# MartinPippel/DAmar

Measured on AMD Instinct MI355X. Metric: aligned base-pairs/sec (daligner block-vs-block), higher is better.
Workload: dtype int32

## Files before the change

damar_amd/csrc/kernels/seed_merge.hip:

```cpp
#include "dev_common.h"
#include "kernels.h"

SEED_PRIO_VAR(g_merge_prio, 0)
SEED_PRIO_SETTER(damar_merge_set_prio, g_merge_prio)


__device__ __forceinline__ u32 count_below(const u32 *__restrict__ bpos, u32 jb, u32 ib, u32 bound)
{ u32 a = jb, b = ib;
  while (a < b)
    { u32 m = (a + b) >> 1;
      if (bpos[m] < bound) a = m + 1; else b = m;
    }
  return a - jb;
}


#ifndef MT_PER
#define MT_PER  4
#endif
#define MT_A    (MT_PER * 256)
#define MT_BCAP (3 * MT_A)
#define MT_HITS 4
#define MT_NBK  2048

// ... 1172 lines not shown
              }
        }
      else
        {
#pragma unroll
          for (int y = 0; y < q; y++)
            prev = (d[y] == d[q]) ? c[y] : prev;
        }
      add[q] = min(c[q] - prev, kmer);
    }
  if (UNS && top > SCREEN_PANEL)
    return true;
  bool ok = false;
#pragma unroll
  for (int x = 0; x < N; x++)
    { int sum = 0;
#pragma unroll
      for (int y = 0; y < N; y++)
        sum += ((u32) (d[y] - d[x]) <= 1u) ? add[y] : 0;
      ok |= (x < n) && (sum >= hitmin);
    }
  return ok;
}

template <bool UNS>
__global__ __launch_bounds__(256)
void pair_work_mark(const u64 *__restrict__ keys, const u32 *__restrict__ vals, u64 nhits, int ppos, int dbits, int abits,
                    int minhit, int nshift, const u64 *__restrict__ send, int binshift, int kmer, int hitmin,
                    u32 b_lo, u32 b_hi, u64 *__restrict__ bits, u32 *__restrict__ tcount)
{ SEED_PRIO(g_merge_prio);
  __shared__ u64 sk[DAMAR_SCAN_TILE + PW_HALO + 1];
  __shared__ u64 bb[(PH_ROUNDS + 1) * 4];
  __shared__ u16 hl[DAMAR_SCAN_TILE];
  __shared__ u16 cl[DAMAR_SCAN_TILE];
  __shared__ u32 kb[DAMAR_SCAN_TILE / 32];
  __shared__ u32 bl[DAMAR_SCAN_TILE / PW_SMALL];
  __shared__ u32 nh, nlo, nhi, nb;
  const int  pshift = ppos + dbits;
  const u64  pmask = (1ull << ppos) - 1;
  const int  nthr = nshift < 0 ? 0 : 1 << nshift;
  const int  l = lane_id(), w = threadIdx.x >> 6;
  const u64  base = (u64) blockIdx.x * DAMAR_SCAN_TILE;
  {
    constexpr int NLD = (DAMAR_SCAN_TILE + PW_HALO + 1 + 255) / 256;
    u64 v[NLD];
#pragma unroll
    for (int q = 0; q < NLD; q++)
      { u64 i = base + (u64) q * 256u + threadIdx.x;
        i = i > 0 ? i - 1 : 0;
        v[q] = keys[i < nhits ? i : nhits - 1];
      }
#pragma unroll
    for (int q = 0; q < NLD; q++)
      { const u32 j = (u32) q * 256u + threadIdx.x;
        if (j < DAMAR_SCAN_TILE + PW_HALO + 1)
          sk[j] = v[q];
      }
  }
  if (threadIdx.x < DAMAR_SCAN_TILE / 32)
    kb[threadIdx.x] = 0;
  if (threadIdx.x == 0)
    nh = nlo = nhi = nb = 0;
  u64 e0 = ~0ull, e1 = ~0ull;
  for (int t = 0; t < nthr; t++)
    { const u64 e = send[t];
      if (e > base)
        { e0 = e;
          if (t + 1 < nthr)
            e1 = send[t + 1];
          break;
        }
    }
  __syncthreads();

  u64 mk[PH_ROUNDS];
  u32 tot = 0;
#pragma unroll
  for (int r = 0; r <= PH_ROUNDS; r++)
    { const u32 off = (u32) r * 256u + threadIdx.x;
      const u64 i = base + off;
      bool st = true, f = false;
      if (i < nhits && off < DAMAR_SCAN_TILE + PW_HALO)
        { const u64 pr = sk[off + 1] >> pshift;
          const u64 ip = i + (u64) (minhit - 1);
          st = (i == 0) || (sk[off] >> pshift) != pr;
          if (r < PH_ROUNDS && st && ip < nhits)
            { const u64 kp = (minhit - 1 <= PW_HALO) ? sk[off + (u32) minhit] : keys[ip];
              if ((kp >> pshift) == pr)
                { f = true;
                  if (i < e0)
                    { if (i + (u64) minhit >= e0) f = false; }
                  else if (i < e1)
                    { if (i + (u64) minhit >= e1) f = false; }
                  else
                    for (int t = 0; t < nthr; t++)
                      { u64 e = send[t];
                        if (i < e)
                          { if (i + (u64) minhit >= e) f = false;
                            break;
                          }
                      }
                }
            }
        }
      const u64 ms = __ballot(st);
      if (l == 0)
        bb[r * 4 + w] = ms;
      if (r < PH_ROUNDS)
        { mk[r] = __ballot(f);
          tot += (u32) __popcll(mk[r]);
        }
    }
  if (tot != 0)
    { u32 at = 0;
      if (l == 0)
        at = atomicAdd(&nh, tot);
      at = (u32) __shfl((int) at, 0);
#pragma unroll
      for (int r = 0; r < PH_ROUNDS; r++)
        { if ((mk[r] >> l) & 1)
            hl[at + (u32) __popcll(mk[r] & lanes_below(l))] = (u16) ((u32) r * 256u + threadIdx.x);
          at += (u32) __popcll(mk[r]);
        }
    }
  __syncthreads();

  const u32 nheads = nh;
  for (u32 h0 = 0; h0 < nheads; h0 += 256)
    { const u32 h = h0 + threadIdx.x;
      u32 off = 0;
      int n = 0, kind = 0;
      if (h < nheads)
        { off = hl[h];
          const u32 rb = (u32) ((sk[off + 1] >> pshift) >> abits);
          if (rb >= b_lo && rb < b_hi)
            { const u32 p = off + 1;
              u64 ws = bb[p >> 6] >> (p & 63);
              if (p & 63)
                ws |= bb[(p >> 6) + 1] << (64 - (p & 63));
              n = ws ? __ffsll((long long) ws) : 65;
              if (n > SCREEN_MAX || minhit > SCREEN_MAX ||
                  (!UNS && (int) ((sk[off + (u32) n] >> dbits) & pmask) > SCREEN_PANEL))
                atomicOr(&kb[off >> 5], 1u << (off & 31));
              else if (n > PW_SMALL)
                bl[atomicAdd(&nb, 1u)] = off | ((u32) n << 16);
              else
                kind = n > PW_SHORT ? 2 : 1;
            }
        }
      const u64 m1 = __ballot(kind == 1), m2 = __ballot(kind == 2);
      u32 a1 = 0, a2 = 0;
      if (l == 0)
        { if (m1) a1 = atomicAdd(&nlo, (u32) __popcll(m1));
          if (m2) a2 = atomicAdd(&nhi, (u32) __popcll(m2));
        }
      a1 = (u32) __shfl((int) a1, 0);
      a2 = (u32) __shfl((int) a2, 0);
      if (kind == 1)
        cl[a1 + (u32) __popcll(m1 & lanes_below(l))] = (u16) (off | ((u32) n << 12));
      else if (kind == 2)
        cl[DAMAR_SCAN_TILE - 1 - (a2 + (u32) __popcll(m2 & lanes_below(l)))] = (u16) (off | ((u32) n << 12));
    }
  __syncthreads();

  const u32 n_lo = nlo, n_hi = nhi;
  const u32 lo_rounds = (n_lo + 255u) & ~255u;
  for (u32 h0 = 0; h0 < lo_rounds + n_hi; h0 += 256)
    { const u32 h = h0 + threadIdx.x;
      const bool act = h0 < lo_rounds ? h < n_lo : h - lo_rounds < n_hi;
      const u32 e = act ? (u32) cl[h0 < lo_rounds ? h : DAMAR_SCAN_TILE - 1 - (h - lo_rounds)] : 0u;
      const u32 off = e & 0xfffu;
      const int n = act ? (int) (e >> 12) : 0;
      bool keep = false;
      if (dbits == 0)
        { const u64 i = base + off;
          int dlast = 0x7fffffff;
          for (int x = 0; x < n && !keep; x++)
            { const int dx = (int) vals[i + (u64) x] >> binshift;
              if (dx == dlast)
                continue;
              dlast = dx;
              int s0 = 0, s1 = 0, p0 = 0, p1 = 0;
              for (int y = 0; y < n; y++)
                { const int dy = (int) vals[i + (u64) y] >> binshift;
                  const int ap = (int) ((sk[off + 1 + (u32) y] >> dbits) & pmask);
                  if (dy == dx)
                    { s0 += (ap - p0 >= kmer) ? kmer : ap - p0;  p0 = ap; }
                  else if (dy == dx + 1)
                    { s1 += (ap - p1 >= kmer) ? kmer : ap - p1;  p1 = ap; }
                }
              keep = s0 + s1 >= hitmin;
            }
        }
      else if (__ballot(n > 0) != 0)
        { if      (__ballot(n > 7) != 0) keep = pw_screen_small<8, UNS>(sk + off + 1, n, pmask, dbits, binshift, kmer, hitmin);
          else if (__ballot(n > 6) != 0) keep = pw_screen_small<7, UNS>(sk + off + 1, n, pmask, dbits, binshift, kmer, hitmin);
          else if (__ballot(n > 5) != 0) keep = pw_screen_small<6, UNS>(sk + off + 1, n, pmask, dbits, binshift, kmer, hitmin);
          else if (__ballot(n > 4) != 0) keep = pw_screen_small<5, UNS>(sk + off + 1, n, pmask, dbits, binshift, kmer, hitmin);
          else if (__ballot(n > 3) != 0) keep = pw_screen_small<4, UNS>(sk + off + 1, n, pmask, dbits, binshift, kmer, hitmin);
          else                           keep = pw_screen_small<3, UNS>(sk + off + 1, n, pmask, dbits, binshift, kmer, hitmin);
        }
      if (keep)
        atomicOr(&kb[off >> 5], 1u << (off & 31));
    }
  const u32 nbig = nb;
  for (u32 q = threadIdx.x >> 6; q < nbig; q += 4)
    { const u32 off = bl[q] & 0xffffu;
      const int n = (int) (bl[q] >> 16);
      const u64 i = base + off;
      const int xl = l < n ? l : n - 1;
      const int dx = seed_diag(sk[off + 1 + (u32) xl], vals, i + (u64) xl, pmask, dbits) >> binshift;
      if (UNS)
        {
          const int apx = (int) ((sk[off + 1 + (u32) xl] >> dbits) & pmask);
          int prev = 0, top = 0;
          for (int y = 0; y < n; y++)
            { const u64 ky = sk[off + 1 + (u32) y];
              const int dy = seed_diag(ky, vals, i + (u64) y, pmask, dbits) >> binshift;
              const int ap = (int) ((ky >> dbits) & pmask);
              const bool before = ap < apx || (ap == apx && y < xl);
              prev = (dy == dx && before && ap > prev) ? ap : prev;
              top = ap > top ? ap : top;
            }
          const int addx = (l < n) ? min(apx - prev, kmer) : 0;
          int sum = 0;
          for (int y = 0; y < n; y++)
            { const int ay = __shfl(addx, y), dy = __shfl(dx, y);
              sum += ((u32) (dy - dx) <= 1u) ? ay : 0;
            }
          if ((top > SCREEN_PANEL || __ballot(l < n && sum >= hitmin) != 0) && l == 0)
            atomicOr(&kb[off >> 5], 1u << (off & 31));
          continue;
        }
      int s0 = 0, s1 = 0, p0 = 0, p1 = 0;
#pragma unroll 4
      for (int y = 0; y < n; y++)
        { const u64 ky = sk[off + 1 + (u32) y];
          const int dy = seed_diag(ky, vals, i + (u64) y, pmask, dbits) >> binshift;
          const int ap = (int) ((ky >> dbits) & pmask);
          if (dy == dx)
            { s0 += (ap - p0 >= kmer) ? kmer : ap - p0;  p0 = ap; }
          else if (dy == dx + 1)
            { s1 += (ap - p1 >= kmer) ? kmer : ap - p1;  p1 = ap; }
        }
      if (__ballot(s0 + s1 >= hitmin) != 0 && l == 0)
        atomicOr(&kb[off >> 5], 1u << (off & 31));
    }
  __syncthreads();
  if (threadIdx.x < 64)
    { const u64 m = (u64) kb[2 * threadIdx.x] | ((u64) kb[2 * threadIdx.x + 1] << 32);
      bits[(base >> 6) + threadIdx.x] = m;
      const int c = wave_incl_scan_i(__popcll(m));
      if (threadIdx.x == 63)
        tcount[blockIdx.x] = (u32) c;
    }
}

#define OR_MAX   2048
#define OR_WAVE  512
#define OR_SLICE 32
__device__ __forceinline__ u32 run_length(const u64 *keys, u64 nhits, u64 i, int pshift, u32 maxrun, int l, u64 pr)
{ u32 n = 0;
  for (;;)
    { const u64 x = i + (u64) n + (u64) l;
      const u64 same = __ballot(x < nhits && (keys[x] >> pshift) == pr);
      if (same != ~0ull)
        return n + (u32) __ffsll((long long) ~same) - 1u;
      n += 64;
      if (n > maxrun)
        return n;
    }
}

__global__ __launch_bounds__(256)
void order_probe(const u64 *__restrict__ keys, u64 nhits, int ppos, int dbits, const u64 *__restrict__ bits, u64 *__restrict__ flag,
                 u32 maxrun)
{ SEED_PRIO(g_merge_prio);
  __shared__ u16 hl[DAMAR_SCAN_TILE];
  __shared__ u32 nh;
  const int  l = lane_id();
  const u64  base = (u64) blockIdx.x * DAMAR_SCAN_TILE;
  if (threadIdx.x == 0)
    nh = 0;
  __syncthreads();
  if (threadIdx.x < DAMAR_SCAN_TILE / 64)
    { u64 w = bits[(base >> 6) + threadIdx.x];
      while (w)
        { const int b = __ffsll((long long) w) - 1;
          w &= w - 1;
          hl[atomicAdd(&nh, 1u)] = (u16) (threadIdx.x * 64u + (u32) b);
        }
    }
  __syncthreads();
  const u32 n_h = nh;
  bool over = false;
  for (u32 h = threadIdx.x >> 6; h < n_h; h += 4)
    { const u64 i = base + hl[h];
      over |= run_length(keys, nhits, i, ppos + dbits, maxrun, l, keys[i] >> (ppos + dbits)) > maxrun;
    }
  if (over && l == 0)
    atomicOr((unsigned long long *) flag, 1ull);
}

template <u32 J>
__device__ __forceinline__ u32 lane_xor(u32 v)
{ if constexpr (J == 1)
    return (u32) __builtin_amdgcn_update_dpp(0, (int) v, 0xB1, 0xf, 0xf, true);
  else if constexpr (J == 2)
    return (u32) __builtin_amdgcn_update_dpp(0, (int) v, 0x4E, 0xf, 0xf, true);
  else if constexpr (J == 8)
    return (u32) __builtin_amdgcn_update_dpp(0, (int) v, 0x128, 0xf, 0xf, true);
  else if constexpr (J == 4 || J == 16)
    return (u32) __builtin_amdgcn_ds_swizzle((int) v, (int) (0x1f | (J << 10)));
  else
    return (u32) __shfl_xor((int) v, (int) J);
}

template <int K, u32 K2, u32 JJ>
__device__ __forceinline__ void or_step(u32 (&c)[K], int l)
{ if constexpr (JJ >= 64)
    {
#pragma unroll
      for (int q = 0; q < K; q++)
        if ((q & (int) (JJ >> 6)) == 0)
          { const int  p  = q | (int) (JJ >> 6);
            const bool up = (((u32) q << 6) & K2) == 0;
            const u32  lo = min(c[q], c[p]), hi = max(c[q], c[p]);
            c[q] = up ? lo : hi;
            c[p] = up ? hi : lo;
          }
    }
  else
    {
#pragma unroll
      for (int q = 0; q < K; q++)
        { const u32  o  = lane_xor<JJ>(c[q]);
          const bool up = (((u32) q * 64u + (u32) l) & K2) == 0;
          c[q] = (up == (((u32) l & JJ) == 0)) ? min(c[q], o) : max(c[q], o);
        }
    }
}

template <int K, u32 K2, u32 JJ>
__device__ __forceinline__ void or_merge(u32 (&c)[K], int l)
{ or_step<K, K2, JJ>(c, l);
  if constexpr (JJ > 1)
    or_merge<K, K2, JJ / 2>(c, l);
}

template <int K, u32 K2>
__device__ __forceinline__ void or_network(u32 (&c)[K], int l)
{ if constexpr (K2 > 2)
    or_network<K, K2 / 2>(c, l);
  or_merge<K, K2, K2 / 2>(c, l);
}

template <int K>
__device__ __forceinline__ void or_sort_regs(u64 *keys, u64 i, u32 n, int dbits, u64 pmask, int l)
{ u32 c[K];
#pragma unroll
  for (int q = 0; q < K; q++)
    { const u32 j = (u32) q * 64u + (u32) l;
      c[q] = (j < n) ? (((u32) ((keys[i + j] >> dbits) & pmask) << 11) | j) : 0xffffffffu;
    }
  or_network<K, 64u * K>(c, l);
  u64 v[K];
#pragma unroll
  for (int q = 0; q < K; q++)
    { const u32 j = (u32) q * 64u + (u32) l;
      v[q] = keys[i + ((j < n) ? (c[q] & 2047u) : 0u)];
    }
  asm volatile("s_waitcnt vmcnt(0)" ::: "memory");
#pragma unroll
  for (int q = 0; q < K; q++)
    { const u32 j = (u32) q * 64u + (u32) l;
      if (j < n)
        keys[i + j] = v[q];
    }
}

#ifdef OR_STATS
static __device__ unsigned long long g_or_hist[16];
#endif

__global__ __launch_bounds__(256)
void order_waves(u64 *keys, u64 nhits, int ppos, int dbits, const u32 *__restrict__ work, u32 nwork, u32 slice,
                 u32 *__restrict__ lcount, u32 *__restrict__ llist)
{ SEED_PRIO(g_merge_prio);
  const int  l = lane_id(), pshift = ppos + dbits;
  const u64  pmask = (1ull << ppos) - 1;
  const u32  first = blockIdx.x * slice;
  const u32  end = min(first + slice, nwork);
  for (u32 t = first + (threadIdx.x >> 6); t < end; t += 4)
    { const u64 i = work[t];
      const u64 x = i + (u64) l;
      const u64 k0 = keys[x < nhits ? x : nhits - 1];
      const u64 pr = (u64) __shfl((long long) (k0 >> pshift), 0);
      const u64 same = __ballot(x < nhits && (k0 >> pshift) == pr);
      u32 n;
      if (same != ~0ull)
        n = (u32) __ffsll((long long) ~same) - 1u;
      else
        n = 64u + run_length(keys, nhits, i + 64u, pshift, OR_MAX - 64u, l, pr);
#ifdef OR_STATS
      if (l == 0)
        { int b = 0;
          while (b < 12 && (2u << b) < n) b += 1;
          atomicAdd(&g_or_hist[n > OR_MAX ? 12 : b], 1ull);
          atomicAdd(&g_or_hist[13], (unsigned long long) n);
        }
#endif
      if (n < 2)
        continue;
      if (n <= 64)
        { u32 c[1] = { (u32) l < n ? (((u32) ((k0 >> dbits) & pmask) << 11) | (u32) l) : 0xffffffffu };
          or_network<1, 64u>(c, l);
          const int src = (int) (c[0] & 63u);
          const u32 lo = (u32) __shfl((int) (u32) k0, src), hi = (u32) __shfl((int) (u32) (k0 >> 32), src);
          if ((u32) l < n)
            keys[x] = ((u64) hi << 32) | lo;
        }
      else if (n <= 128)
        or_sort_regs<2>(keys, i, n, dbits, pmask, l);
      else if (n <= 256)
        or_sort_regs<4>(keys, i, n, dbits, pmask, l);
      else if (n <= OR_WAVE)
        or_sort_regs<8>(keys, i, n, dbits, pmask, l);
      else if (n <= OR_MAX && l == 0)
        { const u32 at = atomicAdd(lcount, 1u);
          llist[2 * at] = (u32) i;
          llist[2 * at + 1] = n;
        }
    }
}

__global__ __launch_bounds__(256)
void order_long(u64 *keys, int ppos, int dbits, const u32 *__restrict__ lcount, const u32 *__restrict__ llist)
{ SEED_PRIO(g_merge_prio);
  __shared__ u64 rk[OR_MAX];
  __shared__ u32 ck[OR_MAX];
  const u64  pmask = (1ull << ppos) - 1;
  const u32  nl = *lcount;
  for (u32 b = blockIdx.x; b < nl; b += gridDim.x)
    { const u64 i = llist[2 * b];
      const u32 n = llist[2 * b + 1];
      u32 P = 2;
      while (P < n)
        P <<= 1;
      for (u32 j = threadIdx.x; j < P; j += 256)
        { if (j < n)
            { const u64 k = keys[i + j];
              rk[j] = k;
              ck[j] = ((u32) ((k >> dbits) & pmask) << 11) | j;
            }
          else
            ck[j] = 0xffffffffu;
        }
      __syncthreads();
      for (u32 k2 = 2; k2 <= P; k2 <<= 1)
        for (u32 jj = k2 >> 1; jj > 0; jj >>= 1)
          { for (u32 t = threadIdx.x; t < (P >> 1); t += 256)
              { const u32 ix = ((t & ~(jj - 1)) << 1) | (t & (jj - 1)), px = ix | jj;
                const bool up = (ix & k2) == 0;
                const u32 a = ck[ix], c = ck[px];
                if ((a > c) == up)
                  { ck[ix] = c;  ck[px] = a; }
              }
            __syncthreads();
          }
      for (u32 j = threadIdx.x; j < n; j += 256)
        keys[i + j] = rk[ck[j] & 2047u];
      __syncthreads();
    }
}

size_t damar_order_runs_scratch_bytes(u64 nhits)
{ return sizeof(u32) * (size_t) (2 * (nhits / (OR_WAVE + 1)) + 2); }

#ifdef OR_STATS
static void or_stats_print(void)
{ unsigned long long h[16];
  if (hipMemcpyFromSymbol(h, HIP_SYMBOL(g_or_hist), sizeof(h)) != hipSuccess)
    return;
  unsigned long long runs = 0;
  for (int b = 0; b <= 12; b++)
    runs += h[b];
  fprintf(stderr, "order_runs: %llu kept runs, %llu seeds in them\n", runs, h[13]);
  for (int b = 0; b <= 12; b++)
    if (h[b])
      fprintf(stderr, "  runs of %5d..%-5d %9llu  (%.3f %%)\n", b == 0 ? 1 : (1 << b) + 1, b == 12 ? 1 << 30 : 2 << b, h[b], 100. * h[b] / runs);
}
#endif

void damar_launch_order_runs(u64 *keys, u64 nhits, int ppos, int dbits, const u32 *work, u32 nwork, void *scratch, hipStream_t st)
{ if (nwork == 0)
    return;
#ifdef OR_STATS
  static int reg = 0;
  if (!reg)
    { reg = 1;  atexit(or_stats_print); }
#endif
  u32 *lcount = (u32 *) scratch;
  HIP_CHECK(hipMemsetAsync(lcount, 0, sizeof(u32), st));
  const u32 slice = std::min<u32>(OR_SLICE, 4u * std::max<u32>(1u, nwork / 2048u));
  hipLaunchKernelGGL(order_waves, dim3((nwork + slice - 1) / slice), dim3(256), 0, st, keys, nhits, ppos, dbits, work, nwork, slice,
                     lcount, lcount + 2);
  if (nhits > OR_WAVE)
    { const u64 most = nhits / (OR_WAVE + 1);
      hipLaunchKernelGGL(order_long, dim3((u32) std::min<u64>(std::min<u64>(nwork, most), 1024)), dim3(256), 0, st, keys, ppos, dbits,
                         (const u32 *) lcount, (const u32 *) (lcount + 2));
    }
}

void damar_launch_pair_work(u64 *keys, const u32 *vals, u64 nhits, u64 off, u64 gtotal, int ppos, int dbits, int abits, int minhit, int nshift,
                            u64 *send, u64 *bits, void *scan_work, u64 *total_dev, int binshift, int kmer, int hitmin,
                            u32 b_lo, u32 b_hi, int unsorted, hipStream_t st)
{ HIP_CHECK(hipMemsetAsync(total_dev, 0, 2 * sizeof(u64), st));
  if (nhits == 0)
    return;
  if (nshift > 6)
    nshift = 6;
  const u32 ntiles = (u32) ((nhits + DAMAR_SCAN_TILE - 1) / DAMAR_SCAN_TILE);
  u32 *tcount = (u32 *) scan_work;
  if (nshift >= 0)
    hipLaunchKernelGGL(slice_ends<u64>, dim3(1), dim3(64), 0, st, keys, nhits, off, gtotal, abits + ppos + dbits, nshift, send);
  if (!unsorted)
    hipLaunchKernelGGL(pair_work_mark<false>, dim3(ntiles), dim3(256), 0, st, (const u64 *) keys, vals, nhits, ppos, dbits, abits, minhit,
                       nshift, (const u64 *) send, binshift, kmer, hitmin, b_lo, b_hi, bits, tcount);
  else
    { hipLaunchKernelGGL(pair_work_mark<true>, dim3(ntiles), dim3(256), 0, st, (const u64 *) keys, vals, nhits, ppos, dbits, abits, minhit,
                         nshift, (const u64 *) send, binshift, kmer, hitmin, b_lo, b_hi, bits, tcount);
      static int maxrun = -1;
      if (maxrun < 0)
        { const char *e = getenv("DAMAR_TEST_RUN_MAX");
          maxrun = (e && atoi(e) >= 2 && atoi(e) <= OR_MAX) ? atoi(e) : OR_MAX;
        }
      hipLaunchKernelGGL(order_probe, dim3(ntiles), dim3(256), 0, st, (const u64 *) keys, nhits, ppos, dbits, (const u64 *) bits, total_dev + 1,
                         (u32) maxrun);
    }
  damar_scan_tile_counts(tcount, ntiles, total_dev, st);
}

void damar_launch_pair_work_expand(const u64 *bits, const void *scan_work, u64 nhits, u32 *work, hipStream_t st)
{ if (nhits == 0)
    return;
  const u32 ntiles = (u32) ((nhits + DAMAR_SCAN_TILE - 1) / DAMAR_SCAN_TILE);
  hipLaunchKernelGGL(pair_heads_expand, dim3(ntiles), dim3(64), 0, st, bits, (const u32 *) scan_work, work);
}

__global__ __launch_bounds__(256)
void compact_u32(const u32 *__restrict__ src, const u32 *__restrict__ keep, const u32 *__restrict__ off, u32 n,
                 u32 *__restrict__ out)
{ u32 i = blockIdx.x * 256u + threadIdx.x;
  if (i < n && keep[i])
    out[off[i]] = src[i];
}

void damar_launch_compact_u32(const u32 *src, const u32 *keep, const u32 *off, u32 n, u32 *out, hipStream_t st)
{ if (n == 0)
    return;
  hipLaunchKernelGGL(compact_u32, dim3((n + 255) / 256), dim3(256), 0, st, src, keep, off, n, out);
}

__global__ __launch_bounds__(256)
void compact_index(const u32 *__restrict__ flags, const u32 *__restrict__ off, u64 n, u32 *__restrict__ out)
{ u64 i = (u64) blockIdx.x * 256u + threadIdx.x;
  if (i < n && flags[i])
    out[off[i]] = (u32) i;
}

void damar_launch_compact_index(const u32 *flags, const u32 *off, u64 n, u32 *out, hipStream_t st)
{ if (n == 0)
    return;
  hipLaunchKernelGGL(compact_index, dim3((u32) ((n + 255) / 256)), dim3(256), 0, st, flags, off, n, out);
}

__global__ __launch_bounds__(256)
void work_cost(const u64 *__restrict__ keys, const u32 *__restrict__ vals, u64 nhits, int pbits0, int abits, int dbits,
               const u32 *__restrict__ aboff, const u32 *__restrict__ bboff,
               const u32 *__restrict__ work, u32 nwork, u32 coarse, u32 *__restrict__ key, u32 *__restrict__ val)
{ u32 j = blockIdx.x * 256u + threadIdx.x;
  if (j >= nwork)
    return;
  const int pbits = pbits0 + dbits;
  const u64 i = work[j], pr = keys[i] >> pbits;
  u64 a = i + 1, b = (j + 1 < nwork) ? (u64) work[j + 1] : nhits;
  while (a < b)
    { u64 mid = (a + b) >> 1;
      if ((keys[mid] >> pbits) == pr) a = mid + 1; else b = mid;
    }
  u64 n = a - i;
  if (coarse >= 0xfffffffcu)
    { const u64 pm = (1ull << pbits0) - 1;
      const u64 ext = ((keys[a - 1] >> dbits) & pm) - ((keys[i] >> dbits) & pm);
      const u32 ra = (u32) (pr & ((1ull << abits) - 1)), rb = (u32) (pr >> abits);
      const int alen = (int) (aboff[ra + 1] - aboff[ra]) - 1, blen = (int) (bboff[rb + 1] - bboff[rb]) - 1;
      const int d = seed_diag(keys[i], vals, i, pm, dbits);
      const int geo = min(alen, blen + d) - max(0, d);
      u64 len = (coarse == 0xffffffffu) ? ext : (coarse == 0xfffffffeu ? (u64) max(geo, 0) : max(ext, (u64) max(geo, 0)));
      if (coarse == 0xfffffffcu)
        { const int xa0 = (int) ((keys[i] >> dbits) & pm), xb0 = xa0 - d;
          const int fw = min(alen - xa0, blen - xb0);
          len = (u64) max(fw, 0);
        }
      n = len >> (pbits0 > 16 ? pbits0 - 16 : 0);
      coarse = 0;
    }
  if (n > WORK_COST_MAX)
    n = WORK_COST_MAX;
  if (coarse == 1)
    key[j] = (u32) __clz((int) n) - (32 - WORK_COST_BITS);
  else
    key[j] = coarse ? (n >= coarse ? 0u : 1u) : (u32) (WORK_COST_MAX - n);
  val[j] = j;
}

void damar_launch_work_cost(const u64 *keys, const u32 *vals, u64 nhits, int pbits, int abits, int dbits, const u32 *aboff,
                            const u32 *bboff, const u32 *work, u32 nwork, u32 coarse, u32 *key, u32 *val, hipStream_t st)
{ if (nwork == 0)
    return;
  hipLaunchKernelGGL(work_cost, dim3((nwork + 255) / 256), dim3(256), 0, st, keys, vals, nhits, pbits, abits, dbits, aboff, bboff,
                     work, nwork, coarse, key, val);
}

void damar_preload_merge(void)
{ hipFuncAttributes fa;
  (void) hipFuncGetAttributes(&fa, (const void *) merge_emit);
}
```

Baseline: 53.83 billion.

## Fuse pair-work marking and run-length probe into one register-staged kernel

Adds a new kernel for the unsorted path that loads each wavefront's keys into registers and detects run boundaries with ballots. It stages the members of short runs into an LDS pool and screens them from there, and it folds the order/run-length overflow check that the separate order_probe kernel used to do into the same pass. This removes one kernel launch and a second sweep over keys and bits, and cuts repeated global reads during screening. The cost is heavy register and LDS use, with occupancy capped at six waves per EU, plus considerable new code that must match the old marking exactly. A fallback to the old two-kernel path remains when DAMAR_WORK_STAGED is set or dbits is zero.

```diff
diff --git a/damar_amd/csrc/kernels/seed_merge.hip b/damar_amd/csrc/kernels/seed_merge.hip
--- a/damar_amd/csrc/kernels/seed_merge.hip
+++ b/damar_amd/csrc/kernels/seed_merge.hip
@@ -1498,6 +1498,272 @@
     atomicOr((unsigned long long *) flag, 1ull);
 }
 
+#define PW_WSEEDS (DAMAR_SCAN_TILE / 4)
+#define PW_POOL   1792
+static_assert(PW_WSEEDS == PH_ROUNDS * 64 && PW_HALO == 64 && SCREEN_MAX < PW_HALO, "a wavefront's rounds and its halo round");
+
+__device__ __forceinline__ u64 lane_before(u64 v, u64 first)
+{ const u32 lo = (u32) __builtin_amdgcn_update_dpp((int) (u32) first, (int) (u32) v, 0x138, 0xf, 0xf, false);
+  const u32 hi = (u32) __builtin_amdgcn_update_dpp((int) (u32) (first >> 32), (int) (u32) (v >> 32), 0x138, 0xf, 0xf, false);
+  return ((u64) hi << 32) | lo;
+}
+
+__device__ __forceinline__ bool pw_screen_wave(const u64 *run, int n, int l, u64 pmask, int dbits, int binshift, int kmer, int hitmin)
+{ const u64 dmask = (1ull << dbits) - 1;
+  const int xl = l < n ? l : n - 1;
+  const u64 kx = run[xl];
+  const int apx = (int) ((kx >> dbits) & pmask);
+  const int dx = (apx - (int) (kx & dmask)) >> binshift;
+  int prev = 0, top = 0;
+  for (int y = 0; y < n; y++)
+    { const u64 ky = run[y];
+      const int ap = (int) ((ky >> dbits) & pmask);
+      const int dy = (ap - (int) (ky & dmask)) >> binshift;
+      const bool before = ap < apx || (ap == apx && y < xl);
+      prev = (dy == dx && before && ap > prev) ? ap : prev;
+      top = ap > top ? ap : top;
+    }
+  const int addx = (l < n) ? min(apx - prev, kmer) : 0;
+  int sum = 0;
+  for (int y = 0; y < n; y++)
+    { const int ay = __shfl(addx, y), dy = __shfl(dx, y);
+      sum += ((u32) (dy - dx) <= 1u) ? ay : 0;
+    }
+  return top > SCREEN_PANEL || __ballot(l < n && sum >= hitmin) != 0;
+}
+
+__device__ __forceinline__ bool pw_screen_lanes(const u64 *run, int n, u64 pmask, int dbits, int binshift, int kmer, int hitmin)
+{ if      (__ballot(n > 7) != 0) return pw_screen_small<8, true>(run, n, pmask, dbits, binshift, kmer, hitmin);
+  else if (__ballot(n > 6) != 0) return pw_screen_small<7, true>(run, n, pmask, dbits, binshift, kmer, hitmin);
+  else if (__ballot(n > 5) != 0) return pw_screen_small<6, true>(run, n, pmask, dbits, binshift, kmer, hitmin);
+  else if (__ballot(n > 4) != 0) return pw_screen_small<5, true>(run, n, pmask, dbits, binshift, kmer, hitmin);
+  else if (__ballot(n > 3) != 0) return pw_screen_small<4, true>(run, n, pmask, dbits, binshift, kmer, hitmin);
+  return pw_screen_small<3, true>(run, n, pmask, dbits, binshift, kmer, hitmin);
+}
+
+__global__ __launch_bounds__(256) __attribute__((amdgpu_waves_per_eu(6)))
+void pair_work_mark_regs(const u64 *__restrict__ keys, u64 nhits, int ppos, int dbits, int abits, int minhit, int nshift,
+                         const u64 *__restrict__ send, int binshift, int kmer, int hitmin, u32 b_lo, u32 b_hi,
+                         u64 *__restrict__ bits, u32 *__restrict__ tcount, u64 *__restrict__ flag, u32 maxrun)
+{ SEED_PRIO(g_merge_prio);
+  __shared__ u64 pool[PW_POOL];
+  __shared__ u64 mw[4][PH_ROUNDS + 1];
+  __shared__ u16 mp[4][PH_ROUNDS + 1];
+  __shared__ u16 cl[DAMAR_SCAN_TILE];
+  __shared__ u32 bl[DAMAR_SCAN_TILE / PW_SMALL];
+  __shared__ u32 kb[DAMAR_SCAN_TILE / 32];
+  __shared__ unsigned long long cnt;
+  __shared__ u32 inkeys[4];
+  const int  pshift = ppos + dbits;
+  const u64  pmask = (1ull << ppos) - 1;
+  const int  nthr = nshift < 0 ? 0 : 1 << nshift;
+  const int  l = lane_id(), w = threadIdx.x >> 6;
+  const u64  base = (u64) blockIdx.x * DAMAR_SCAN_TILE;
+  const u32  wb = (u32) w * PW_WSEEDS;
+  if (threadIdx.x == 0)
+    cnt = 0;
+  u64 e0 = ~0ull, e1 = ~0ull;
+  for (int t = 0; t < nthr; t++)
+    { const u64 e = send[t];
+      if (e > base)
+        { e0 = e;
+          if (t + 1 < nthr)
+            e1 = send[t + 1];
+          break;
+        }
+    }
+  __syncthreads();
+
+  u64 v[PH_ROUNDS + 1];
+#pragma unroll
+  for (int q = 0; q <= PH_ROUNDS; q++)
+    { const u64 i = base + wb + (u32) q * 64u + (u32) l;
+      v[q] = keys[i < nhits ? i : nhits - 1];
+    }
+  u64 ms[PH_ROUNDS + 1];
+  { const u64 ib = base + wb;
+    u64 last = keys[ib == 0 ? 0 : (ib - 1 < nhits ? ib - 1 : nhits - 1)];
+#pragma unroll
+    for (int q = 0; q <= PH_ROUNDS; q++)
+      { const u64 i = ib + (u32) q * 64u + (u32) l;
+        const u64 d = (v[q] ^ lane_before(v[q], last)) >> pshift;
+        ms[q] = __ballot(i >= nhits || i == 0 || d != 0);
+        last = bcast_u64(v[q], 63);
+      }
+  }
+
+  u32 code[(PH_ROUNDS + 1 + 3) / 4];
+  u32 n1 = 0, n2 = 0, n3 = 0, npool = 0;
+  u32 carry = 0;
+  bool over = false;
+#pragma unroll
+  for (int x = 0; x < (PH_ROUNDS + 1 + 3) / 4; x++)
+    code[x] = 0;
+#pragma unroll
+  for (int q = 0; q <= PH_ROUNDS; q++)
+    { u64 scr = 0;
+      u32 c = 0;
+      if (q < PH_ROUNDS)
+        { const u32 off = wb + (u32) q * 64u + (u32) l;
+          const u64 i = base + off;
+          u64 ws = ((ms[q] >> 1) >> l) | (ms[q + 1] << (63 - l));
+          const int n = ws ? __ffsll((long long) ws) : 65;
+          bool f = ((ms[q] >> l) & 1) && i < nhits && n >= (minhit - 1 > PW_HALO ? PW_HALO + 1 : minhit);
+          if (minhit - 1 > PW_HALO)
+            { const u64 ip = i + (u64) (minhit - 1);
+              f = f && ip < nhits;
+              if (f)
+                f = (keys[ip] >> pshift) == (v[q] >> pshift);
+            }
+          if (f)
+            { if (i < e0)
+                { if (i + (u64) minhit >= e0) f = false; }
+              else if (i < e1)
+                { if (i + (u64) minhit >= e1) f = false; }
+              else
+                for (int t = 0; t < nthr; t++)
+                  { u64 e = send[t];
+                    if (i < e)
+                      { if (i + (u64) minhit >= e) f = false;
+                        break;
+                      }
+                  }
+              const u32 rb = (u32) ((v[q] >> pshift) >> abits);
+              if (rb < b_lo || rb >= b_hi)
+                f = false;
+            }
+          const bool direct = f && (n > SCREEN_MAX || minhit > SCREEN_MAX);
+          const u64 kd = __ballot(direct);
+          if (l == 0)
+            { kb[(wb >> 5) + 2 * q] = (u32) kd;
+              kb[(wb >> 5) + 2 * q + 1] = (u32) (kd >> 32);
+            }
+          over |= direct && (u32) n > maxrun && (n <= 64 || maxrun < 64);
+          u64 lm = __ballot(direct && n > 64 && maxrun >= 64);
+          while (lm)
+            { const int b = __ffsll((long long) lm) - 1;
+              lm &= lm - 1;
+              const u64 ih = base + wb + (u32) q * 64u + (u32) b;
+              over |= run_length(keys, nhits, ih, pshift, maxrun, l, bcast_u64(v[q], b) >> pshift) > maxrun;
+            }
+          if (f && !direct)
+            c = (u32) n;
+          scr = __ballot(c != 0);
+          n1 += (u32) __popcll(__ballot(c != 0 && c <= PW_SHORT));
+          n2 += (u32) __popcll(__ballot(c > PW_SHORT && c <= PW_SMALL));
+          n3 += (u32) __popcll(__ballot(c > PW_SMALL));
+        }
+      const u64 a = ~(ms[q] & ~scr), s1 = a + scr, sum = s1 + carry;
+      const u32 cout = (s1 < a || sum < s1) ? 1u : 0u;
+      const u64 mem = ((sum ^ a ^ scr) >> 1) | ((u64) cout << 63);
+      carry = cout;
+      npool += (u32) __popcll(mem);
+      c |= (u32) ((mem >> l) & 1) << 7;
+      code[q >> 2] |= c << (8 * (q & 3));
+    }
+  if (__ballot(over) != 0 && l == 0)
+    atomicOr((unsigned long long *) flag, 1ull);
+
+  u32 a1, a2, a3, ap;
+  bool staged;
+  { unsigned long long at = 0;
+    if (l == 0)
+      at = atomicAdd(&cnt, (unsigned long long) n1 | ((unsigned long long) n2 << 16) | ((unsigned long long) n3 << 32) |
+                           ((unsigned long long) npool << 48));
+    at = bcast_u64(at, 0);
+    a1 = (u32) at & 0xffffu;  a2 = (u32) (at >> 16) & 0xffffu;  a3 = (u32) (at >> 32) & 0xffffu;  ap = (u32) (at >> 48);
+    staged = ap + npool <= PW_POOL;
+    if (l == 0)
+      inkeys[w] = staged ? 0u : 1u;
+  }
+  u64 my_mw = 0;
+  u32 my_mp = 0;
+#pragma unroll
+  for (int q = 0; q <= PH_ROUNDS; q++)
+    { const u32 c = (code[q >> 2] >> (8 * (q & 3))) & 0xffu;
+      const u32 n = c & 0x7fu, off = wb + (u32) q * 64u + (u32) l;
+      const u64 mem = __ballot((c & 0x80u) != 0);
+      if (l == q)
+        { my_mw = mem;  my_mp = ap; }
+      if (staged && (c & 0x80u))
+        pool[ap + (u32) __popcll(mem & lanes_below(l))] = v[q];
+      ap += (u32) __popcll(mem);
+      if (q < PH_ROUNDS)
+        { const u64 m1 = __ballot(n != 0 && n <= PW_SHORT), m2 = __ballot(n > PW_SHORT && n <= PW_SMALL), m3 = __ballot(n > PW_SMALL);
+          if (m1)
+            { if (n != 0 && n <= PW_SHORT)
+                cl[a1 + (u32) __popcll(m1 & lanes_below(l))] = (u16) (off | (n << 12));
+              a1 += (u32) __popcll(m1);
+            }
+          if (m2)
+            { if (n > PW_SHORT && n <= PW_SMALL)
+                cl[DAMAR_SCAN_TILE - 1 - (a2 + (u32) __popcll(m2 & lanes_below(l)))] = (u16) (off | (n << 12));
+              a2 += (u32) __popcll(m2);
+            }
+          if (m3)
+            { if (n > PW_SMALL)
+                bl[a3 + (u32) __popcll(m3 & lanes_below(l))] = off | (n << 16);
+              a3 += (u32) __popcll(m3);
+            }
+        }
+    }
+  if (l <= PH_ROUNDS)
+    { mw[w][l] = my_mw;
+      mp[w][l] = (u16) my_mp;
+    }
+  __syncthreads();
+
+  const unsigned long long tot = cnt;
+  const u32 n_lo = (u32) tot & 0xffffu, n_hi = (u32) (tot >> 16) & 0xffffu, nbig = (u32) (tot >> 32) & 0xffffu;
+  const u32 lo_rounds = (n_lo + 255u) & ~255u;
+  over = false;
+  for (u32 h0 = 0; h0 < lo_rounds + n_hi; h0 += 256)
+    { const u32 h = h0 + threadIdx.x;
+      const bool act = h0 < lo_rounds ? h < n_lo : h - lo_rounds < n_hi;
+      const u32 e = act ? (u32) cl[h0 < lo_rounds ? h : DAMAR_SCAN_TILE - 1 - (h - lo_rounds)] : 0u;
+      const u32 off = e & 0xfffu;
+      const int n = act ? (int) (e >> 12) : 0;
+      if (__ballot(n > 0) == 0)
+        continue;
+      const u32 hw = off >> 10, hq = (off >> 6) & (PH_ROUNDS - 1), hb = off & 63u;
+      bool keep;
+      if (__ballot(act && inkeys[hw] != 0) != 0)
+        keep = pw_screen_lanes(keys + base + off, n, pmask, dbits, binshift, kmer, hitmin);
+      else
+        keep = pw_screen_lanes(pool + (act ? (u32) mp[hw][hq] + (u32) __popcll(mw[hw][hq] & lanes_below((int) hb)) : 0u), n, pmask,
+                               dbits, binshift, kmer, hitmin);
+      if (keep)
+        { atomicOr(&kb[off >> 5], 1u << (off & 31));
+          over |= (u32) n > maxrun;
+        }
+    }
+  for (u32 q = threadIdx.x >> 6; q < nbig; q += 4)
+    { const u32 off = bl[q] & 0xffffu;
+      const int n = (int) (bl[q] >> 16);
+      const u32 hw = off >> 10, hq = (off >> 6) & (PH_ROUNDS - 1), hb = off & 63u;
+      bool keep;
+      if (inkeys[hw] != 0)
+        keep = pw_screen_wave(keys + base + off, n, l, pmask, dbits, binshift, kmer, hitmin);
+      else
+        keep = pw_screen_wave(pool + (u32) mp[hw][hq] + (u32) __popcll(mw[hw][hq] & lanes_below((int) hb)), n, l, pmask, dbits,
+                              binshift, kmer, hitmin);
+      if (keep && l == 0)
+        { atomicOr(&kb[off >> 5], 1u << (off & 31));
+          over |= (u32) n > maxrun;
+        }
+    }
+  if (__ballot(over) != 0 && l == 0)
+    atomicOr((unsigned long long *) flag, 1ull);
+  __syncthreads();
+  if (threadIdx.x < 64)
+    { const u64 m = (u64) kb[2 * threadIdx.x] | ((u64) kb[2 * threadIdx.x + 1] << 32);
+      bits[(base >> 6) + threadIdx.x] = m;
+      const int c = wave_incl_scan_i(__popcll(m));
+      if (threadIdx.x == 63)
+        tcount[blockIdx.x] = (u32) c;
+    }
+}
+
 template <u32 J>
 __device__ __forceinline__ u32 lane_xor(u32 v)
 { if constexpr (J == 1)
@@ -1724,15 +1990,22 @@
     hipLaunchKernelGGL(pair_work_mark<false>, dim3(ntiles), dim3(256), 0, st, (const u64 *) keys, vals, nhits, ppos, dbits, abits, minhit,
                        nshift, (const u64 *) send, binshift, kmer, hitmin, b_lo, b_hi, bits, tcount);
   else
-    { hipLaunchKernelGGL(pair_work_mark<true>, dim3(ntiles), dim3(256), 0, st, (const u64 *) keys, vals, nhits, ppos, dbits, abits, minhit,
-                         nshift, (const u64 *) send, binshift, kmer, hitmin, b_lo, b_hi, bits, tcount);
-      static int maxrun = -1;
+    { static int maxrun = -1;
+      static int staged = 0;
       if (maxrun < 0)
         { const char *e = getenv("DAMAR_TEST_RUN_MAX");
           maxrun = (e && atoi(e) >= 2 && atoi(e) <= OR_MAX) ? atoi(e) : OR_MAX;
-        }
-      hipLaunchKernelGGL(order_probe, dim3(ntiles), dim3(256), 0, st, (const u64 *) keys, nhits, ppos, dbits, (const u64 *) bits, total_dev + 1,
-                         (u32) maxrun);
+          staged = (e = getenv("DAMAR_WORK_STAGED")) != NULL && atoi(e) != 0;
+        }
+      if (dbits != 0 && !staged)
+        hipLaunchKernelGGL(pair_work_mark_regs, dim3(ntiles), dim3(256), 0, st, (const u64 *) keys, nhits, ppos, dbits, abits, minhit,
+                           nshift, (const u64 *) send, binshift, kmer, hitmin, b_lo, b_hi, bits, tcount, total_dev + 1, (u32) maxrun);
+      else
+        { hipLaunchKernelGGL(pair_work_mark<true>, dim3(ntiles), dim3(256), 0, st, (const u64 *) keys, vals, nhits, ppos, dbits, abits,
+                             minhit, nshift, (const u64 *) send, binshift, kmer, hitmin, b_lo, b_hi, bits, tcount);
+          hipLaunchKernelGGL(order_probe, dim3(ntiles), dim3(256), 0, st, (const u64 *) keys, nhits, ppos, dbits, (const u64 *) bits,
+                             total_dev + 1, (u32) maxrun);
+        }
     }
   damar_scan_tile_counts(tcount, ntiles, total_dev, st);
 }
```

Measured after the change: 53.89 billion, median of 2. No clear change (+0.1%).
